# TropComplique/MultiPoseNet

Hardware: AMD Instinct MI355X
Metric: images/sec keypoint fwd+bwd+Adam @512x512 bs32/GPU (higher is better)
Workload: dtype bf16; 1 GPU; MobileNet-v1+FPN+keypoint_subnet fwd+bwd+Adam, 512x512, per-GPU batch 32; global_batch=32, parallelism=dp1, hip_graph=True, rccl_ranks=1

## Files before the change

### include/mpn.h

```cpp
#ifndef MPN_H_
#define MPN_H_

#include <stddef.h>
#include <stdint.h>

#ifdef __cplusplus
extern "C" {
#endif

#define MPN_VERSION 600

enum { MPN_F32 = 0, MPN_BF16 = 1, MPN_F16 = 2  };

enum {
    MPN_OK = 0,
    MPN_ERR_BAD_SHAPE = -1,
    MPN_ERR_BAD_DTYPE = -2,
    MPN_ERR_BAD_ALIGN = -3,
    MPN_ERR_HIP = -4,
    MPN_ERR_BAD_ARG = -5,
    MPN_ERR_WORKSPACE = -6,
    MPN_ERR_BAD_DATA = -7
};

// ... 138 lines not shown
                               mpn_stream_t stream);
int mpn_dwconv_bwd_fused_s2_apply(const void* x, const void* g, const void* y_raw, const float* w, void* dx, float* wpart, int N, int H,
                                  int W, int C, int dtype, const float* in_scale, const float* in_shift, int in_act,
                                  const float* mean, const float* invstd, float* bn_part, const void* addend, const float* ap_scale,
                                  const float* ap_shift, const float* ap_mean, const float* ap_invstd, const float* ap_k1,
                                  const float* ap_k2, int ap_act, mpn_stream_t stream);

int mpn_stem_conv_fwd(const void* images, int images_u8, const float* w, void* y, int N, int H,
                      int W, int C0, int dtype, mpn_stream_t stream);
int mpn_stem_conv_fwd_num_parts(int N, int H, int W, int C0, int dtype);
int mpn_stem_conv_fwd_stats(const void* images, int images_u8, const float* w, void* y, int N, int H, int W, int C0,
                            int dtype, float* stats_part, mpn_stream_t stream);
int mpn_stem_conv_wgrad_num_parts(int N, int H, int W);
int mpn_stem_conv_bwd_weight(const void* images, int images_u8, const void* dy, float* part, int N,
                             int H, int W, int C0, int dtype, mpn_stream_t stream);

int mpn_bilinear_up_fwd(const void* x, void* y, int N, int h, int w, int C, int upsample,
                        int y_channel_offset, int y_channels_total, int dtype,
                        const float* in_scale, const float* in_shift, int in_act,
                        mpn_stream_t stream);
int mpn_bilinear_up_bwd(const void* dy, void* dx, int N, int h, int w, int C, int upsample,
                        int y_channel_offset, int y_channels_total, int dtype, mpn_stream_t stream);
int mpn_sumpool2x2(const void* src, void* dst, int N, int h, int w, int C, int accumulate,
                   int dtype, mpn_stream_t stream);
int mpn_add_inplace(void* dst, const void* src, long long n, int dtype, mpn_stream_t stream);

int mpn_heatmap_head_fwd(const void* x, const float* w, const float* bias, long long M, int Cin,
                         int dtype, const float* in_scale, const float* in_shift, int in_act,
                         int mode, float* out, float* out_seg, mpn_stream_t stream);
int mpn_heatmap_head_bwd_num_parts(long long M);
// ... 426 lines not shown
```

### multiposenet_amd/_lib.py

```python
import ctypes
import os

_HERE = os.path.dirname(os.path.abspath(__file__))
LIB_PATH = os.environ.get("MPN_LIB") or os.path.join(_HERE, "libmpn_hip.so")

MPN_VERSION = 600
MPN_F32, MPN_BF16, MPN_F16 = 0, 1, 2
ACT_NONE, ACT_RELU, ACT_RELU6 = 0, 1, 2

_c = ctypes
_P = _c.c_void_p
_I = _c.c_int
_F = _c.c_float
_D = _c.c_double
_Z = _c.c_size_t
_L = _c.c_longlong

SIGNATURES = {
    "mpn_version": (_I, []),
    "mpn_last_error": (_I, [_c.c_char_p, _Z]),
    "mpn_heatmap_decode_workspace_bytes": (_Z, [_I]),
    "mpn_heatmap_decode": (_I, [_P, _I, _I, _I, _I, _I, _P, _F, _P, _P, _P, _P, _Z, _P]),
    "mpn_heatmap_render_workspace_bytes": (_Z, [_I]),
    "mpn_heatmap_render": (_I, [_P, _P, _P, _I, _I, _I, _I, _I, _P, _P, _Z, _P]),
# ... 38 lines not shown
    "mpn_dwconv_bwd_data_add_supported": (_I, [_I, _I, _I, _I, _I, _I]),
    "mpn_dwconv_bwd_data_add": (_I, [_P, _P, _P, _I, _I, _I, _I, _I, _I, _P, _P, _P, _P, _P, _P, _I, _P, _P]),
    "mpn_dwconv_wgrad_num_parts": (_I, [_I, _I, _I, _I, _I, _I]),
    "mpn_dwconv_bwd_weight": (_I, [_P, _P, _P, _I, _I, _I, _I, _I, _I, _P, _P, _I, _P]),
    "mpn_dwconv_bwd_fused_supported": (_I, [_I, _I, _I, _I, _I, _I]),
    "mpn_dwconv_bwd_fused": (_I, [_P, _P, _P, _P, _P, _I, _I, _I, _I, _I, _P, _P, _I, _P, _P, _P, _P]),
    "mpn_dwconv_bwd_fused_s2": (_I, [_P, _P, _P, _P, _P, _I, _I, _I, _I, _I, _P, _P, _I, _P, _P, _P, _P, _P]),
    "mpn_dwconv_bwd_fused_apply_supported": (_I, [_I, _I, _I, _I, _I, _I]),
    "mpn_dwconv_bwd_fused_apply": (_I, [_P, _P, _P, _P, _P, _P, _I, _I, _I, _I, _I, _P, _P, _I, _P, _P, _P, _P, _P, _P, _P, _P, _P, _I, _P]),
    "mpn_dwconv_bwd_fused_s2_apply": (_I, [_P, _P, _P, _P, _P, _P, _I, _I, _I, _I, _I, _P, _P, _I, _P, _P, _P, _P, _P, _P, _P, _P, _P, _P, _I, _P]),
    "mpn_stem_conv_fwd": (_I, [_P, _I, _P, _P, _I, _I, _I, _I, _I, _P]),
    "mpn_stem_conv_fwd_num_parts": (_I, [_I, _I, _I, _I, _I]),
    "mpn_stem_conv_fwd_stats": (_I, [_P, _I, _P, _P, _I, _I, _I, _I, _I, _P, _P]),
    "mpn_stem_conv_wgrad_num_parts": (_I, [_I, _I, _I]),
    "mpn_stem_conv_bwd_weight": (_I, [_P, _I, _P, _P, _I, _I, _I, _I, _I, _P]),
    "mpn_bilinear_up_fwd": (_I, [_P, _P, _I, _I, _I, _I, _I, _I, _I, _I, _P, _P, _I, _P]),
    "mpn_bilinear_up_bwd": (_I, [_P, _P, _I, _I, _I, _I, _I, _I, _I, _I, _P]),
    "mpn_sumpool2x2": (_I, [_P, _P, _I, _I, _I, _I, _I, _I, _P]),
    "mpn_add_inplace": (_I, [_P, _P, _L, _I, _P]),
    "mpn_heatmap_head_fwd": (_I, [_P, _P, _P, _L, _I, _I, _P, _P, _I, _I, _P, _P, _P]),
    "mpn_heatmap_head_bwd_num_parts": (_I, [_L]),
    "mpn_heatmap_head_bwd": (_I, [_P, _P, _P, _L, _I, _I, _P, _P, _I, _P, _P, _P]),
    "mpn_heatmap_head_bwd_bn_supported": (_I, [_I, _I]),
    "mpn_heatmap_head_bwd_bn": (_I, [_P, _P, _P, _L, _I, _I, _P, _P, _I, _P, _P, _P, _P]),
    "mpn_keypoint_loss_num_parts": (_I, [_I, _I, _I]),
    "mpn_keypoint_loss": (_I, [_P] * 9 + [_I, _I] + [_P] * 7 + [_I, _I, _I, _P]),
    "mpn_adam_prepare": (_I, [_P, _P, _D, _D, _D, _D, _D, _P]),
    "mpn_adam_step": (_I, [_P, _P, _P, _P, _L, _P, _F, _F, _F, _F, _F, _P]),
    "mpn_adam_step_cast": (_I, [_P, _P, _P, _P, _L, _P, _F, _F, _F, _F, _F, _I, _P, _P, _P, _I, _P]),
    "mpn_reduce_partials": (_I, [_P, _I, _L, _P, _I, _F, _P]),
# ... 237 lines not shown
```

### multiposenet_amd/csrc/conv_mfma.hip

```cpp
#include "common.h"
#include "pointwise.h"
#include "conv3x3.h"
#include <type_traits>
#include <string.h>

namespace {

typedef __bf16 bf16x8_t __attribute__((ext_vector_type(8)));
typedef __bf16 bf16x4_t __attribute__((ext_vector_type(4)));
typedef float f32x4_t __attribute__((ext_vector_type(4)));
typedef float f32x16_t __attribute__((ext_vector_type(16)));

template <typename T> struct Mma;
template <> struct Mma<bf16_t> {
    using Frag = bf16x8_t;
    static __device__ __forceinline__ void run(const Frag& a, const Frag& b, f32x4_t& c) {
        c = __builtin_amdgcn_mfma_f32_16x16x32_bf16(a, b, c, 0, 0, 0);
    }
};
template <> struct Mma<half_t> {
    using Frag = H16<half_t>::x8;
    static __device__ __forceinline__ void run(const Frag& a, const Frag& b, f32x4_t& c) { c = H16<half_t>::mfma(a, b, c); }
};
template <> struct Mma<float> {
// ... 600 lines not shown
    constexpr int EPS = 16 / ES;
    const int q = e / EPS, within = e - q * EPS;
    const long long dst = i - e + (long long)((q ^ b_swz(n & 15)) * EPS + within);
    out[dst] = from_f32<T>(v);
}

template <typename T>
__global__ void pack_weights_kernel(const float* __restrict__ w, T* __restrict__ out, int Cin_o, int Cout_o,
                                    int taps, int transpose, int BN, int n_tiles, int nchunk, int row_bytes,
                                    long long total_elems) {
    for (long long i = (long long)blockIdx.x * blockDim.x + threadIdx.x; i < total_elems;
         i += (long long)gridDim.x * blockDim.x)
        pack_one<T>(w, out, Cin_o, Cout_o, taps, transpose, BN, nchunk, row_bytes, i);
}

template <typename T>
__global__ void pack_weights_batched_kernel(const PackDesc* __restrict__ descs, int ndesc) {
    __shared__ int job;
    if (threadIdx.x < 64) {
        int cnt = 0;
        for (int base = 0; base < ndesc; base += 64) {
            const int i = base + (int)threadIdx.x;
            const bool le = i < ndesc && descs[i].block_begin <= (int)blockIdx.x;
            cnt += __popcll(__ballot(le));
        }
        if (threadIdx.x == 0) job = cnt - 1;
    }
    __syncthreads();
    const PackDesc d = descs[job];
    const int lb = blockIdx.x - d.block_begin;
    for (long long i = (long long)lb * blockDim.x + threadIdx.x; i < d.total_elems; i += (long long)d.block_count * blockDim.x)
        pack_one<T>(d.w, reinterpret_cast<T*>(d.out), d.Cin_o, d.Cout_o, d.taps, d.transpose, d.BN, d.nchunk, d.row_bytes, i);
}

struct PackGeom {
    int BN, n_tiles, nchunk, row_bytes;
    long long tile_bytes, total_bytes;
};

PackGeom pack_geom(int Kin, int Nout, int taps, int es, int dtype) {
    PackGeom g;
    if (dtype == MPN_BF16 && pw_gemm_eligible(Kin, Nout, taps, es)) {
        g.BN = 256; g.n_tiles = Nout / 256; g.nchunk = 1; g.row_bytes = 0;
        g.tile_bytes = 256ll * Kin * es; g.total_bytes = (long long)Nout * Kin * es;
        return g;
// ... 47 lines not shown

extern "C" size_t mpn_conv_pack_desc_bytes(void) { return sizeof(PackDesc); }

extern "C" int mpn_conv_pack_desc_fill(void* desc_host, const float* w_hwio, int Cin, int Cout, int ksize, int transpose,
                                       int dtype, void* out, int block_begin) {
    if (!(ksize == 1 || ksize == 3) || !desc_host || !w_hwio || !out) return -1;
    const int es = dtype == MPN_F32 ? 4 : 2;
    const int taps = ksize * ksize;
    const PackGeom g = pack_geom(transpose ? Cout : Cin, transpose ? Cin : Cout, taps, es, dtype);
    PackDesc d;
    d.w = w_hwio; d.out = out; d.Cin_o = Cin; d.Cout_o = Cout; d.taps = taps; d.transpose = transpose;
    d.BN = g.BN; d.n_tiles = g.n_tiles; d.nchunk = g.nchunk; d.row_bytes = g.row_bytes;
    d.total_elems = g.total_bytes / es;
    long long blocks = (d.total_elems + 4 * 256 - 1) / (4 * 256);
    if (blocks > 256) blocks = 256;
    if (blocks < 1) blocks = 1;
    d.block_begin = block_begin;
    d.block_count = (int)blocks;
    memcpy(desc_host, &d, sizeof(d));
    return (int)blocks;
}

extern "C" int mpn_conv_pack_weights_batched(const void* descs_device, int ndesc, int total_blocks, int dtype,
                                             mpn_stream_t stream) {
    MPN_REQUIRE(descs_device && ndesc > 0 && total_blocks > 0, MPN_ERR_BAD_ARG, "pack batched: bad arguments");
    MPN_REQUIRE(dtype == MPN_F32 || dtype == MPN_BF16 || dtype == MPN_F16, MPN_ERR_BAD_DTYPE, "pack batched: dtype");
    hipStream_t st = (hipStream_t)stream;
    MPN_DISPATCH_DTYPE3(dtype, (pack_weights_batched_kernel<T><<<total_blocks, 256, 0, st>>>((const PackDesc*)descs_device, ndesc)));
    MPN_LAUNCH_CHECK();
    return MPN_OK;
// ... 271 lines not shown
```

### multiposenet_amd/csrc/stem.hip

```cpp
#include "common.h"

namespace {

constexpr int kThreads = 256;
constexpr int kTile = 16;
constexpr int kIn = 2 * kTile + 1;
constexpr int kMaxC0 = 64;
constexpr int kFwdTW = 2 * kTile;

template <typename T, bool U8>
__device__ __forceinline__ void stage_patch(const void* images, float* patch, int img, int oy0, int ox0, int H, int W,
                                            int pad_t, int pad_l) {
    const int iy0 = oy0 * 2 - pad_t, ix0 = ox0 * 2 - pad_l;
    constexpr int NEL = kIn * kIn * 3;
    constexpr int PER = (NEL + kThreads - 1) / kThreads;
    float v[PER];
#pragma unroll
    for (int k = 0; k < PER; ++k) {
        const int i = threadIdx.x + k * kThreads;
        const int ch = i % 3;
        const int px = (i / 3) % kIn;
        const int py = i / (3 * kIn);
        const int iy = iy0 + py, ix = ix0 + px;
        float raw = 0.5f;
// ... 222 lines not shown
        const int r = wv * 4 + (gi >> 1), col = (gi & 1) * 16 + n;
        unsigned char* dst = otile + (r * kFwdTW + col) * orow + (4 * kg) * 2;
#pragma unroll
        for (int mb = 0; mb < MB; ++mb) {
            const acc_t c = acc[gi][mb];
            uint2 q;
            q.x = pack_bf16x2(c[0], c[1]);
            q.y = pack_bf16x2(c[2], c[3]);
            *reinterpret_cast<uint2*>(dst + mb * 32) = q;
        }
    }
    __syncthreads();
    stem_copy_out<bf16_t>(otile, orow, y, img, ty, tx, OH, OW, C0, stats_part);
}

template <typename T, bool U8>
__global__ __launch_bounds__(kThreads) void stem_wgrad_kernel(const void* __restrict__ images, const T* __restrict__ dy,
                                                              float* __restrict__ part, int N, int H, int W, int C0, int OH,
                                                              int OW, int pad_t, int pad_l, int tiles_x, int tiles_y) {
    extern __shared__ __attribute__((aligned(16))) float dyn_smem[];
    float* patch = dyn_smem;
    float* g = dyn_smem + kIn * kIn * 3 + 1;
    const int ncq = C0 / 8;
    const int tpp = 9 * ncq;
    const int nphase = min(kThreads / tpp, kTile * kTile / 27);
    const int ph = threadIdx.x / tpp;
    const int r = threadIdx.x - ph * tpp;
    const int pos = r / ncq, cq = r - pos * ncq;
    const int ky = pos / 3, kx = pos - ky * 3;
    const bool active = ph < nphase;
    f32x2_t acc[3][4];
#pragma unroll
    for (int a = 0; a < 3; ++a)
#pragma unroll
        for (int j = 0; j < 4; ++j) acc[a][j] = (f32x2_t){0.f, 0.f};
    const int nout = 27 * C0;
    const int ntiles = N * tiles_y * tiles_x;
    constexpr int NEL = kIn * kIn * 3;
    constexpr int PER = (NEL + kThreads - 1) / kThreads;
    constexpr int VE = Vec16<T>::N;
    constexpr int DPER = kTile * kTile * (kMaxC0 / VE) / kThreads;
    const int vpp = C0 / VE;
    const int ndv = kTile * kTile * vpp / kThreads;
    float pv[PER];
    Vec16<T> dvv[DPER];
    unsigned pmask = 0u, dmask = 0u;

    auto load_tile = [&](int t) {
        const int tx = t % tiles_x;
        const int t2 = t / tiles_x;
        const int ty = t2 % tiles_y;
        const int img = t2 / tiles_y;
        const int oy0 = ty * kTile, ox0 = tx * kTile;
        const int iy0 = oy0 * 2 - pad_t, ix0 = ox0 * 2 - pad_l;
        pmask = 0u;
        dmask = 0u;
#pragma unroll
        for (int k = 0; k < PER; ++k) {
            const int i = threadIdx.x + k * kThreads;
            const int ch = i % 3;
            const int px = (i / 3) % kIn;
            const int py = i / (3 * kIn);
            const int iy = iy0 + py, ix = ix0 + px;
            const bool ok = i < NEL && iy >= 0 && iy < H && ix >= 0 && ix < W;
            const long long off = ok ? (((long long)img * H + iy) * W + ix) * 3 + ch : 0;
            pv[k] = U8 ? (float)reinterpret_cast<const unsigned char*>(images)[off] * (1.0f / 255.0f)
                       : reinterpret_cast<const float*>(images)[off];
            pmask |= (ok ? 1u : 0u) << k;
        }
#pragma unroll
        for (int k = 0; k < DPER; ++k) {
            if (k < ndv) {
                const int i = threadIdx.x + k * kThreads;
                const int vq = i % vpp, px = i / vpp;
                const int oy = oy0 + px / kTile, ox = ox0 + px % kTile;
                const bool ok = oy < OH && ox < OW;
                dvv[k].load(dy + (ok ? (((long long)img * OH + oy) * OW + ox) * C0 + vq * VE : 0));
                dmask |= (ok ? 1u : 0u) << k;
            }
        }
    };
    auto commit_tile = [&]() {
#pragma unroll
        for (int k = 0; k < PER; ++k) {
            const int i = threadIdx.x + k * kThreads;
            if (i < NEL) patch[i] = ((pmask >> k) & 1u) ? 2.0f * pv[k] - 1.0f : 0.0f;
        }
#pragma unroll
        for (int k = 0; k < DPER; ++k) {
            if (k < ndv) {
                const int i = threadIdx.x + k * kThreads;
                const int vq = i % vpp, px = i / vpp;
                float f[VE];
                dvv[k].unpack(f);
                const bool ok = (dmask >> k) & 1u;
#pragma unroll
                for (int j = 0; j < VE; j += 4)
                    *reinterpret_cast<float4*>(g + px * C0 + vq * VE + j) =
                        ok ? make_float4(f[j], f[j + 1], f[j + 2], f[j + 3]) : make_float4(0.f, 0.f, 0.f, 0.f);
            }
        }
    };

    int t = blockIdx.x;
    if (t < ntiles) {
        load_tile(t);
        commit_tile();
    }
// ... 27 lines not shown
        for (int a = 0; a < 3; ++a)
#pragma unroll
            for (int j = 0; j < 4; ++j) {
                g[ph * nout + (pos * 3 + a) * C0 + cq * 8 + 2 * j] = acc[a][j].x;
                g[ph * nout + (pos * 3 + a) * C0 + cq * 8 + 2 * j + 1] = acc[a][j].y;
            }
    }
    __syncthreads();
    for (int o = threadIdx.x; o < nout; o += kThreads) {
        float s = 0.f;
        for (int q = 0; q < nphase; ++q) s += g[q * nout + o];
        part[(long long)blockIdx.x * nout + o] = s;
    }
}

template <bool U8, int MB>
__global__ __launch_bounds__(kThreads) void stem_wgrad_mfma_kernel(const void* __restrict__ images, const bf16_t* __restrict__ dy,
                                                                   float* __restrict__ part, int N, int H, int W, int OH, int OW,
                                                                   int pad_t, int pad_l, int tiles_x, int tiles_y) {
    typedef H16<bf16_t> HT;
    typedef HT::x8 x8;
    typedef HT::x4 x4;
    typedef HT::acc_t acc_t;
    constexpr int C0 = 16 * MB;
    constexpr int DRS = C0 * 2 + 16;
    extern __shared__ __attribute__((aligned(16))) unsigned char stem_smem[];
    float* patch = reinterpret_cast<float*>(stem_smem);
    unsigned char* dimg = stem_smem + kPR * kPS * sizeof(float);
    const int ntiles = N * tiles_y * tiles_x;
    const int lane = threadIdx.x & 63, wv = threadIdx.x >> 6;
    const int n = lane & 15, kg = lane >> 4, q = n >> 2, pq = n & 3;
    constexpr int VPP = C0 / 8;
    constexpr int DV = kTile * kFwdTW * VPP / kThreads;
    float pv[kPR];
    uint4 dv[DV];
    unsigned long long pmask = 0ull;
    unsigned dmask = 0u;
    const int p_pc = threadIdx.x < kPC ? threadIdx.x : 0;
    auto load_tile = [&](int t) __attribute__((always_inline)) {
        const int tx = t % tiles_x;
        const int t2 = t / tiles_x;
        const int ty = t2 % tiles_y;
        const int img = t2 / tiles_y;
        const int iy0 = ty * kTile * 2 - pad_t, ix0 = tx * kFwdTW * 2 - pad_l;
        pmask = 0ull;
        dmask = 0u;
        int tid = threadIdx.x;
        asm volatile("" : "+v"(tid));
        {
            const int ix = ix0 + p_pc / 3;
            const bool col_ok = tid < kPC && ix >= 0 && ix < W;
            const long long base = ((long long)img * H * W + ix0) * 3 + p_pc;
#pragma unroll
            for (int py = 0; py < kPR; ++py) {
                const int iy = iy0 + py;
                const bool ok = col_ok && iy >= 0 && iy < H;
                const long long off = ok ? base + (long long)iy * W * 3 : 0;
                pv[py] = U8 ? (float)reinterpret_cast<const unsigned char*>(images)[off] * (1.0f / 255.0f)
                            : reinterpret_cast<const float*>(images)[off];
                pmask |= (unsigned long long)(ok ? 1u : 0u) << py;
            }
        }
#pragma unroll
        for (int k = 0; k < DV; ++k) {
            const int i = tid + k * kThreads;
            const int vq = i % VPP, px = i / VPP;
            const int oy = ty * kTile + px / kFwdTW, ox = tx * kFwdTW + px % kFwdTW;
            const bool ok = oy < OH && ox < OW;
            dv[k] = *reinterpret_cast<const uint4*>(dy + (ok ? (((long long)img * OH + oy) * OW + ox) * C0 + vq * 8 : 0));
            dmask |= (ok ? 1u : 0u) << k;
        }
    };
    auto commit_tile = [&]() __attribute__((always_inline)) {
        int tid = threadIdx.x;
        asm volatile("" : "+v"(tid));
        if (tid < kPC) {
#pragma unroll
            for (int py = 0; py < kPR; ++py)
                patch[py * kPS + p_pc] = ((pmask >> py) & 1ull) ? 2.0f * pv[py] - 1.0f : 0.0f;
        }
#pragma unroll
        for (int k = 0; k < DV; ++k) {
            const int i = tid + k * kThreads;
            const int vq = i % VPP, px = i / VPP;
            *reinterpret_cast<uint4*>(dimg + px * DRS + vq * 16) = ((dmask >> k) & 1u) ? dv[k] : make_uint4(0u, 0u, 0u, 0u);
        }
    };
    int kbase[2];
    bool kval[2];
#pragma unroll
    for (int nb = 0; nb < 2; ++nb) {
        const int k = nb * 16 + n;
        kval[nb] = k < 27;
        kbase[nb] = kval[nb] ? (k / 9) * kPS + (k % 9) : 0;
    }
    acc_t acc[MB][2];
#pragma unroll
    for (int mb = 0; mb < MB; ++mb)
#pragma unroll
        for (int nb = 0; nb < 2; ++nb) acc[mb][nb] = (acc_t){0.f, 0.f, 0.f, 0.f};
// ... 48 lines not shown
        for (int nb = 0; nb < 2; ++nb)
            *reinterpret_cast<float4*>(red + ((wv * (MB * 2) + mb * 2 + nb) * 64 + lane) * 4) =
                make_float4(acc[mb][nb][0], acc[mb][nb][1], acc[mb][nb][2], acc[mb][nb][3]);
    __syncthreads();
    for (int o = threadIdx.x; o < 27 * C0; o += kThreads) {
        const int k = o / C0, co = o - k * C0;
        const int nb = k >> 4, nn = k & 15, mb = co >> 4, m = co & 15;
        const int ln = (m >> 2) * 16 + nn, e = m & 3;
        float sacc = 0.f;
#pragma unroll
        for (int w4 = 0; w4 < 4; ++w4) sacc += red[((w4 * (MB * 2) + mb * 2 + nb) * 64 + ln) * 4 + e];
        part[(long long)blockIdx.x * (27 * C0) + o] = sacc;
    }
}

template <bool U8, int MB>
int launch_stem_wgrad_mfma(int grid, hipStream_t st, const void* images, const void* dy, float* part, int N, int H, int W, int OH,
                           int OW, int pt, int pl, int tiles_x, int tiles_y) {
    constexpr int sm = kPR * kPS * (int)sizeof(float) + kTile * kFwdTW * (16 * MB * 2 + 16);
    static mpn_attr_mask_t attr_mask{0};
    MPN_HIP(mpn_ensure_dynamic_lds((const void*)stem_wgrad_mfma_kernel<U8, MB>, sm, &attr_mask));
    stem_wgrad_mfma_kernel<U8, MB><<<grid, kThreads, sm, st>>>(images, (const bf16_t*)dy, part, N, H, W, OH, OW, pt, pl, tiles_x, tiles_y);
    return MPN_OK;
}

void same_pad(int size, int* out, int* pad_before) {
    *out = (size + 1) / 2;
    int total = (*out - 1) * 2 + 3 - size;
    if (total < 0) total = 0;
    *pad_before = total / 2;
}

int check(int N, int H, int W, int C0, int dtype) {
    MPN_REQUIRE(dtype == MPN_F32 || dtype == MPN_BF16, MPN_ERR_BAD_DTYPE, "stem: dtype %d", dtype);
    const int ve = dtype == MPN_F32 ? 4 : 8;
    MPN_REQUIRE(N > 0 && H > 0 && W > 0, MPN_ERR_BAD_SHAPE, "stem: bad shape");
    MPN_REQUIRE(C0 > 0 && C0 <= kMaxC0 && C0 % ve == 0, MPN_ERR_BAD_SHAPE, "stem: C0 (%d) must be <= %d and a multiple of %d",
                C0, kMaxC0, ve);
// ... 58 lines not shown
        } else {
            if (sm > 48 * 1024)
                MPN_HIP(hipFuncSetAttribute((const void*)stem_fwd_kernel<T, false>, hipFuncAttributeMaxDynamicSharedMemorySize, sm));
            stem_fwd_kernel<T, false><<<grid, kThreads, sm, st>>>(images, w, (T*)y, N, H, W, C0, OH, OW, pt, pl, tiles_x, tiles_y, stats_part);
        }
    });
    MPN_LAUNCH_CHECK();
    return MPN_OK;
}

extern "C" int mpn_stem_conv_wgrad_num_parts(int N, int H, int W) {
    const int ntiles = N * (((H + 1) / 2 + kTile - 1) / kTile) * (((W + 1) / 2 + kTile - 1) / kTile);
    return ntiles < 512 ? ntiles : 512;
}

extern "C" int mpn_stem_conv_bwd_weight(const void* images, int images_u8, const void* dy, float* part, int N, int H, int W,
                                        int C0, int dtype, mpn_stream_t stream) {
    if (int rc = check(N, H, W, C0, dtype)) return rc;
    MPN_REQUIRE(images && dy && part, MPN_ERR_BAD_ARG, "stem_wgrad: null pointer");
    int OH, OW, pt, pl;
    same_pad(H, &OH, &pt);
    same_pad(W, &OW, &pl);
    const int tiles_y = (OH + kTile - 1) / kTile, tiles_x = (OW + kTile - 1) / kTile;
    const int grid = mpn_stem_conv_wgrad_num_parts(N, H, W);
    hipStream_t st = (hipStream_t)stream;
    MPN_REQUIRE(C0 % 8 == 0, MPN_ERR_BAD_SHAPE, "stem_wgrad: C0 must be a multiple of 8");
    if (dtype == MPN_BF16 && C0 % 16 == 0) {
        const int tx32 = (OW + kFwdTW - 1) / kFwdTW;
        int rc;
#define MPN_STEM_WG(MB)                                                                                                         \
    rc = images_u8 ? launch_stem_wgrad_mfma<true, MB>(grid, st, images, dy, part, N, H, W, OH, OW, pt, pl, tx32, tiles_y)       \
                   : launch_stem_wgrad_mfma<false, MB>(grid, st, images, dy, part, N, H, W, OH, OW, pt, pl, tx32, tiles_y)
        switch (C0 / 16) {
            case 1: MPN_STEM_WG(1); break;
            case 2: MPN_STEM_WG(2); break;
            case 3: MPN_STEM_WG(3); break;
            default: MPN_STEM_WG(4); break;
        }
#undef MPN_STEM_WG
        if (rc) return rc;
        MPN_LAUNCH_CHECK();
        return MPN_OK;
    }
    const size_t sm = (size_t)(kIn * kIn * 3 + 1 + kTile * kTile * C0) * sizeof(float);
    MPN_REQUIRE(sm <= 64 * 1024, MPN_ERR_BAD_SHAPE, "stem_wgrad: C0 too large");
    MPN_DISPATCH_DTYPE(dtype, {
        if (images_u8)
            stem_wgrad_kernel<T, true><<<grid, kThreads, sm, st>>>(images, (const T*)dy, part, N, H, W, C0, OH, OW, pt, pl, tiles_x, tiles_y);
        else
            stem_wgrad_kernel<T, false><<<grid, kThreads, sm, st>>>(images, (const T*)dy, part, N, H, W, C0, OH, OW, pt, pl, tiles_x, tiles_y);
    });
    MPN_LAUNCH_CHECK();
    return MPN_OK;
}
```

### multiposenet_amd/net.py

```python
import math
import os
from collections import OrderedDict

import numpy as np
import torch

from . import _lib, ops
from ._lib import ACT_NONE, ACT_RELU, ACT_RELU6
from .model_state import ModelState, _Arena, is_trainable, resolve_device

NUM_KEYPOINTS = 17
DOWNSAMPLE = 4
DIVISOR = 128
DEPTH = 128
STRIDES_AND_FILTERS = [(1, 64), (2, 128), (1, 128), (2, 256), (1, 256), (2, 512), (1, 512), (1, 512),
                       (1, 512), (1, 512), (1, 512), (2, 1024), (1, 1024)]
FEATURE_BLOCKS = {3: "c2", 5: "c3", 11: "c4", 13: "c5"}


def depth(x, depth_multiplier):
    return max(int(x * depth_multiplier), 8)


def variable_shapes(depth_multiplier=1.0):
# ... 132 lines not shown
                               conv2=self._conv(s + "/conv2/kernel"), bn2=self._bn(s + "/bn2", ACT_RELU))
        self.final_conv = self._conv("final_conv3x3/kernel")
        self.final_bn = self._bn("final_bn", ACT_RELU)
        self.concat_scale = torch.ones(4 * DEPTH, dtype=torch.float32, device=self.device)
        self.concat_shift = torch.zeros(4 * DEPTH, dtype=torch.float32, device=self.device)
        self.phi[2]["bn2"].scale = self.concat_scale[:DEPTH]
        self.phi[2]["bn2"].shift = self.concat_shift[:DEPTH]
        self.concat_affine = ops.Affine(self.concat_scale, self.concat_shift, ACT_RELU)
        self.heat_w, self.heat_b = self.vars["heatmaps/kernel"], self.vars["heatmaps/bias"]
        ok, nk, _ = self._train_arena.offsets["heatmaps/kernel"]
        ob, nb, _ = self._train_arena.offsets["heatmaps/bias"]
        assert ob == ok + nk, "heatmaps/kernel and heatmaps/bias must be adjacent in the arena"
        self._head_grad = self.grad[ok:ob + nb]
        self.fuse_dw_bn = True
        self.fuse_dw_apply = True
        self.fuse_conv_bn = True
        self._l2 = None
        self._wd = None
        self.cache_inference_affine = False
        self._infer_clean = False
        self.fuse_stem_stats = True
        self._build_pack_table()
        self.all_bn = [self.stem_bn] + [b[k] for b in self.blocks for k in ("dw_bn", "pw_bn")] + \
            [self.p_bn[l] for l in (2, 3, 4, 5)] + [self.phi[l][k] for l in (2, 3, 4, 5) for k in ("bn1", "bn2")] + [self.final_bn]

    def _build_pack_table(self):
        import ctypes
        lib = ops._lib.lib()
        nb = lib.mpn_conv_pack_desc_bytes()
        jobs = [(c, t) for c in self.convs for t in (0, 1)]
# ... 368 lines not shown
        if phase == 1:
            dA, reduced, lateral_added = g["c"]["c5"], g.get("c5_reduced", 0), False
            rng = range(last, first - 1, -1)
        else:
            dA, reduced, lateral_added = g["bb_chain"]
            rng = range(first - 1, -1, -1)
        for i in rng:
            feature = FEATURE_BLOCKS.get(self.blocks[i]["i"])
            if feature in ("c2", "c3", "c4") and not lateral_added:
                ops.add_inplace(dA, g["c"][feature])
            dY, applied = self._backward_pointwise(b, g, sp, slab, i, dA, reduced, raw=i == last, fold=self._dw_folds_apply(b, g, i))
            dA, reduced, lateral_added = self._backward_depthwise(b, g, sp, slab, i, dY, apply=not applied)
        if phase == 1:
            g["bb_chain"] = (dA, reduced, lateral_added)
            return
        ops.bn_backward(self.stem_bn, g["stem"], b["stem"], sp, reduced_parts=reduced)
        ops.stem_conv_bwd_weight(images, g["stem"], self.stem_dw, slab[id(self.stem_dw)], reduce=False)

    def _dw_lateral(self, g, i):
        return g["c"][FEATURE_BLOCKS[self.blocks[i - 1]["i"]]] if i > 0 and self.blocks[i - 1]["i"] in FEATURE_BLOCKS else None

    def _dw_walks_fused(self, b, g, i):
        s, (N, _, _, C) = self.blocks[i]["stride"], b["dw"][i].shape
        return (self.fuse_dw_bn and (s == 2 or self._dw_lateral(g, i) is None)
                and ops.dwconv_bwd_fused_supported(N, *b["hw"][i], C, s, self.dtype))

    def _dw_folds_apply(self, b, g, i):
        s, (N, _, _, C) = self.blocks[i]["stride"], b["dw"][i].shape
        return (self.fuse_dw_apply and self._dw_walks_fused(b, g, i)
                and ops.dwconv_bwd_fused_apply_supported(N, *b["hw"][i], C, s, self.dtype))

    def _backward_pointwise(self, b, g, sp, slab, i, dA, reduced, raw, fold=False):
# ... 59 lines not shown
```

### multiposenet_amd/ops.py

```python
import ctypes
from collections import namedtuple

import torch

from . import _lib
from ._lib import ACT_NONE, ACT_RELU, ACT_RELU6, call, ptr, stream_ptr

BN_MOMENTUM = 0.95
BN_EPSILON = 1e-3

LAUNCH_JOBS_ALONE = False

Affine = namedtuple("Affine", ["scale", "shift", "act"])


def _f32(n, dev):
    return torch.empty(n, dtype=torch.float32, device=dev)


def _check_nhwc(x, name="x"):
    if x.dim() != 4 or not x.is_contiguous():
        raise ValueError(f"{name} must be a contiguous NHWC tensor, got shape {tuple(x.shape)}")
    if x.dtype not in (torch.float32, torch.bfloat16):
        raise ValueError(f"{name}: unsupported dtype {x.dtype}")
# ... 531 lines not shown
        raise ValueError("images must be float32 in [0,1] or uint8")
    N, H, W, _ = images.shape
    if out is None:
        out = torch.empty((N, (H + 1) // 2, (W + 1) // 2, c0), dtype=dtype, device=images.device)
    if stats_part is not None:
        rows = stem_conv_fwd_num_parts(N, H, W, c0, dtype)
        if rows <= 0 or stats_part.numel() < rows * 2 * c0:
            raise ValueError("stem_conv_fwd: fused statistics not available for this shape, or slab too small")
        call("mpn_stem_conv_fwd_stats", ptr(images), int(u8), ptr(w), ptr(out), N, H, W, c0, _lib.dtype_code(dtype),
             ptr(stats_part), stream_ptr())
        return out
    call("mpn_stem_conv_fwd", ptr(images), int(u8), ptr(w), ptr(out), N, H, W, c0, _lib.dtype_code(dtype), stream_ptr())
    return out


def stem_conv_bwd_weight(images, dy, dw_out, part=None, reduce=True):
    N, H, W, _ = images.shape
    c0 = dy.shape[3]
    nparts = _lib.lib().mpn_stem_conv_wgrad_num_parts(N, H, W)
    if part is None:
        part = _f32(nparts * 27 * c0, dy.device)
    call("mpn_stem_conv_bwd_weight", ptr(images), int(images.dtype == torch.uint8), ptr(dy), ptr(part), N, H, W, c0,
         _lib.dtype_code(dy.dtype), stream_ptr())
    if reduce:
        call("mpn_reduce_partials", ptr(part), nparts, 27 * c0, ptr(dw_out), 0, 1.0, stream_ptr())
    return dw_out


def bilinear_up_fwd(x, upsample, out, channel_offset, affine=None):
    N, h, w, C = x.shape
    sc, sh, act = _aff(affine)
    call("mpn_bilinear_up_fwd", ptr(x), ptr(out), N, h, w, C, upsample, channel_offset, out.shape[3],
         _lib.dtype_code(x.dtype), sc, sh, act, stream_ptr())
    return out


def bilinear_up_bwd(dy, upsample, channel_offset, C, out=None):
    N, OH, OW, ctot = dy.shape
# ... 193 lines not shown
```

Baseline: 4295 images/s.

## Fold stem BN-backward apply into stem weight-grad load; tile weight packing via LDS

The stem batch-norm backward no longer runs a separate apply pass over the stem gradient. The stem weight-gradient kernels now read the raw pre-BN output alongside dy and apply the ReLU mask and BN correction on load, which saves one read/write pass over a large full-resolution activation. Separately, bf16 weight packing now stages 32-row groups through shared memory so that global loads and stores are vectorised and coalesced. The cost is extra register pressure and an additional y load inside the stem wgrad kernel.

Measured after the change: 4320 images/s (median of 6 runs). No clear change (+0.6%).

```diff
diff --git a/include/mpn.h b/include/mpn.h
--- a/include/mpn.h
+++ b/include/mpn.h
@@ -176,6 +176,10 @@
 int mpn_stem_conv_wgrad_num_parts(int N, int H, int W);
 int mpn_stem_conv_bwd_weight(const void* images, int images_u8, const void* dy, float* part, int N,
                              int H, int W, int C0, int dtype, mpn_stream_t stream);
+int mpn_stem_conv_bwd_weight_apply_supported(int N, int H, int W, int C0, int dtype);
+int mpn_stem_conv_bwd_weight_apply(const void* images, int images_u8, const void* g, const void* y_raw, float* part, int N, int H,
+                                   int W, int C0, int dtype, const float* ap_scale, const float* ap_shift, const float* ap_mean,
+                                   const float* ap_invstd, const float* ap_k1, const float* ap_k2, int ap_act, mpn_stream_t stream);
 
 int mpn_bilinear_up_fwd(const void* x, void* y, int N, int h, int w, int C, int upsample,
                         int y_channel_offset, int y_channels_total, int dtype,
diff --git a/multiposenet_amd/_lib.py b/multiposenet_amd/_lib.py
--- a/multiposenet_amd/_lib.py
+++ b/multiposenet_amd/_lib.py
@@ -76,6 +76,8 @@
     "mpn_stem_conv_fwd_stats": (_I, [_P, _I, _P, _P, _I, _I, _I, _I, _I, _P, _P]),
     "mpn_stem_conv_wgrad_num_parts": (_I, [_I, _I, _I]),
     "mpn_stem_conv_bwd_weight": (_I, [_P, _I, _P, _P, _I, _I, _I, _I, _I, _P]),
+    "mpn_stem_conv_bwd_weight_apply_supported": (_I, [_I, _I, _I, _I, _I]),
+    "mpn_stem_conv_bwd_weight_apply": (_I, [_P, _I, _P, _P, _P, _I, _I, _I, _I, _I, _P, _P, _P, _P, _P, _P, _I, _P]),
     "mpn_bilinear_up_fwd": (_I, [_P, _P, _I, _I, _I, _I, _I, _I, _I, _I, _P, _P, _I, _P]),
     "mpn_bilinear_up_bwd": (_I, [_P, _P, _I, _I, _I, _I, _I, _I, _I, _I, _P]),
     "mpn_sumpool2x2": (_I, [_P, _P, _I, _I, _I, _I, _I, _I, _P]),
diff --git a/multiposenet_amd/csrc/conv_mfma.hip b/multiposenet_amd/csrc/conv_mfma.hip
--- a/multiposenet_amd/csrc/conv_mfma.hip
+++ b/multiposenet_amd/csrc/conv_mfma.hip
@@ -638,8 +638,107 @@
         pack_one<T>(w, out, Cin_o, Cout_o, taps, transpose, BN, nchunk, row_bytes, i);
 }
 
+constexpr int kPackGroupK = 32;
+__host__ __device__ inline int pack_group_rows(int BN, int row_bytes) { return row_bytes == 0 ? 64 : BN; }
+
+template <typename T>
+__device__ __forceinline__ void pack_group(const PackDesc& d, int grp, float* __restrict__ tile) {
+    static_assert(sizeof(T) == 2, "tiled packing: 16-bit images");
+    const int Kin = d.transpose ? d.Cout_o : d.Cin_o, Nout = d.transpose ? d.Cin_o : d.Cout_o;
+    const int NB = pack_group_rows(d.BN, d.row_bytes);
+    const int pitch = NB + 4;
+    int tap, cbase, nbase, g = grp;
+    long long dst0 = (long long)grp * NB * kPackGroupK;
+    int dst_pitch = kPackGroupK;
+    if (d.row_bytes == -2) {
+        const int ks = g % 2; g /= 2;
+        const int ky = g % 3; g /= 3;
+        const int kx = g % 3; g /= 3;
+        const int chunk = g % d.nchunk; g /= d.nchunk;
+        tap = ky * 3 + kx; cbase = chunk * 64 + ks * 32; nbase = g * 64;
+    } else if (d.row_bytes < 0) {
+        const int ky = g % 3; g /= 3;
+        const int ks = g % 2; g /= 2;
+        const int kx = g % 3; g /= 3;
+        const int chunk = g % d.nchunk; g /= d.nchunk;
+        tap = ky * 3 + kx; cbase = chunk * 64 + ks * 32; nbase = g * 128;
+    } else if (d.row_bytes == 0) {
+        const int kblocks = Kin / kPackGroupK;
+        const int kb = g % kblocks; g /= kblocks;
+        tap = 0; cbase = kb * kPackGroupK; nbase = g * 64;
+        dst0 = (long long)nbase * Kin + cbase;
+        dst_pitch = Kin;
+    } else {
+        const int stages_per_tap = d.row_bytes >> 7;
+        const int ks = g % 2; g /= 2;
+        const int st = g % stages_per_tap; g /= stages_per_tap;
+        tap = g % d.taps; g /= d.taps;
+        const int chunk = g % d.nchunk; g /= d.nchunk;
+        cbase = chunk * (d.row_bytes / 2) + (st * 2 + ks) * kPackGroupK; nbase = g * d.BN;
+    }
+    const bool swizzled = d.row_bytes != 0;
+    const bool c3 = d.row_bytes < 0;
+    const float* __restrict__ w = d.w;
+    const bool vec_ok = (d.Cout_o & 3) == 0 && (reinterpret_cast<uintptr_t>(w) & 15u) == 0;
+    T* __restrict__ out = reinterpret_cast<T*>(d.out);
+    const int tid = threadIdx.x, nthreads = blockDim.x;
+    if (!d.transpose) {
+        const long long src0 = (long long)tap * d.Cin_o * d.Cout_o;
+        const int f4_per_row = NB / 4;
+        for (int f = tid; f < kPackGroupK * f4_per_row; f += nthreads) {
+            const int row = f / f4_per_row, c4 = f - row * f4_per_row;
+            const int c = cbase + row, co = nbase + c4 * 4;
+            float4 v = make_float4(0.f, 0.f, 0.f, 0.f);
+            if (c < Kin) {
+                const float* src = w + src0 + (long long)c * d.Cout_o + co;
+                if (vec_ok && co + 3 < Nout) v = *reinterpret_cast<const float4*>(src);
+                else {
+                    if (co < Nout) v.x = src[0];
+                    if (co + 1 < Nout) v.y = src[1];
+                    if (co + 2 < Nout) v.z = src[2];
+                    if (co + 3 < Nout) v.w = src[3];
+                }
+            }
+            *reinterpret_cast<float4*>(tile + row * pitch + c4 * 4) = v;
+        }
+        __syncthreads();
+    }
+    for (int vi = tid; vi < NB * 4; vi += nthreads) {
+        const int n = vi >> 2, qd = vi & 3;
+        const int q = swizzled ? (qd ^ (c3 ? mpn_c3::swz(n & 15) : b_swz(n & 15))) : qd;
+        float f[8];
+        if (!d.transpose) {
+#pragma unroll
+            for (int j = 0; j < 8; ++j) f[j] = tile[(q * 8 + j) * pitch + n];
+        } else {
+            const int co = nbase + n, c0 = cbase + q * 8;
+#pragma unroll
+            for (int j = 0; j < 8; ++j) f[j] = 0.f;
+            if (co < Nout) {
+                const float* src = w + ((long long)(d.taps - 1 - tap) * d.Cin_o + co) * d.Cout_o + c0;
+                if (vec_ok && c0 + 7 < Kin) {
+                    const float4 a = *reinterpret_cast<const float4*>(src), b = *reinterpret_cast<const float4*>(src + 4);
+                    f[0] = a.x; f[1] = a.y; f[2] = a.z; f[3] = a.w; f[4] = b.x; f[5] = b.y; f[6] = b.z; f[7] = b.w;
+                } else {
+#pragma unroll
+                    for (int j = 0; j < 8; ++j)
+                        if (c0 + j < Kin) f[j] = src[j];
+                }
+            }
+        }
+        T t[8];
+#pragma unroll
+        for (int j = 0; j < 8; ++j) t[j] = from_f32<T>(f[j]);
+        uint4 o;
+        __builtin_memcpy(&o, t, 16);
+        *reinterpret_cast<uint4*>(out + dst0 + (long long)n * dst_pitch + qd * 8) = o;
+    }
+    if (!d.transpose) __syncthreads();
+}
+
 template <typename T>
 __global__ void pack_weights_batched_kernel(const PackDesc* __restrict__ descs, int ndesc) {
+    __shared__ __attribute__((aligned(16))) float tile[sizeof(T) == 2 ? kPackGroupK * (128 + 4) : 4];
     __shared__ int job;
     if (threadIdx.x < 64) {
         int cnt = 0;
@@ -653,6 +752,13 @@
     __syncthreads();
     const PackDesc d = descs[job];
     const int lb = blockIdx.x - d.block_begin;
+    if constexpr (sizeof(T) == 2) {
+        if ((reinterpret_cast<uintptr_t>(d.out) & 15u) == 0) {
+            const int ngroups = (int)(d.total_elems / (pack_group_rows(d.BN, d.row_bytes) * kPackGroupK));
+            for (int grp = lb; grp < ngroups; grp += d.block_count) pack_group<T>(d, grp, tile);
+            return;
+        }
+    }
     for (long long i = (long long)lb * blockDim.x + threadIdx.x; i < d.total_elems; i += (long long)d.block_count * blockDim.x)
         pack_one<T>(d.w, reinterpret_cast<T*>(d.out), d.Cin_o, d.Cout_o, d.taps, d.transpose, d.BN, d.nchunk, d.row_bytes, i);
 }
@@ -730,6 +836,10 @@
     d.total_elems = g.total_bytes / es;
     long long blocks = (d.total_elems + 4 * 256 - 1) / (4 * 256);
     if (blocks > 256) blocks = 256;
+    if (es == 2) {
+        blocks = d.total_elems / (pack_group_rows(g.BN, g.row_bytes) * kPackGroupK);
+        if (blocks > 512) blocks = 512;
+    }
     if (blocks < 1) blocks = 1;
     d.block_begin = block_begin;
     d.block_count = (int)blocks;
diff --git a/multiposenet_amd/csrc/stem.hip b/multiposenet_amd/csrc/stem.hip
--- a/multiposenet_amd/csrc/stem.hip
+++ b/multiposenet_amd/csrc/stem.hip
@@ -1,8 +1,7 @@
-#include "common.h"
+#include "dwconv_walk.h"
 
 namespace {
 
-constexpr int kThreads = 256;
 constexpr int kTile = 16;
 constexpr int kIn = 2 * kTile + 1;
 constexpr int kMaxC0 = 64;
@@ -260,10 +259,55 @@
     stem_copy_out<bf16_t>(otile, orow, y, img, ty, tx, OH, OW, C0, stats_part);
 }
 
-template <typename T, bool U8>
+struct StemApplyArgs {
+    const void* y;
+    const float* scale; const float* shift; const float* mean; const float* invstd; const float* k1; const float* k2;
+    int act;
+};
+struct StemDyApply {
+    DyApply<bf16_t> a[2];
+    f32x2_t sh[4];
+    float lo, hi;
+    __device__ __forceinline__ void load(const StemApplyArgs& p, int c0) {
+#pragma unroll
+        for (int h = 0; h < 2; ++h) {
+            a[h].load(p.scale, p.mean, p.invstd, p.k1, p.k2, c0 + 4 * h);
+            const float4 h4 = *reinterpret_cast<const float4*>(p.shift + c0 + 4 * h);
+            sh[2 * h] = (f32x2_t){h4.x, h4.y};
+            sh[2 * h + 1] = (f32x2_t){h4.z, h4.w};
+        }
+        lo = (p.act != MPN_ACT_NONE) ? 0.f : -INFINITY;
+        hi = (p.act == MPN_ACT_RELU6) ? 6.f : INFINITY;
+    }
+    __device__ __forceinline__ uint4 apply(const uint4& g, const uint4& y, unsigned elem) const {
+        const unsigned gw[4] = {g.x, g.y, g.z, g.w}, yw[4] = {y.x, y.y, y.z, y.w};
+        unsigned ow[4];
+#pragma unroll
+        for (int h = 0; h < 2; ++h) {
+            const Raw4<bf16_t> gr = {make_uint2(gw[2 * h], gw[2 * h + 1])}, yr = {make_uint2(yw[2 * h], yw[2 * h + 1])};
+            float f[4];
+            raw_unpack(gr, f);
+            f32x2_t y01, y23;
+            raw_unpack2(yr, y01, y23);
+            const f32x2_t p01 = __builtin_elementwise_fma(y01, a[h].sc01, sh[2 * h]);
+            const f32x2_t p23 = __builtin_elementwise_fma(y23, a[h].sc23, sh[2 * h + 1]);
+            f[0] = (p01.x > lo && p01.x < hi) ? f[0] : 0.f;
+            f[1] = (p01.y > lo && p01.y < hi) ? f[1] : 0.f;
+            f[2] = (p23.x > lo && p23.x < hi) ? f[2] : 0.f;
+            f[3] = (p23.y > lo && p23.y < hi) ? f[3] : 0.f;
+            a[h].apply(f, yr, elem);
+            ow[2 * h] = (__float_as_uint(f[0]) >> 16) | (__float_as_uint(f[1]) & 0xffff0000u);
+            ow[2 * h + 1] = (__float_as_uint(f[2]) >> 16) | (__float_as_uint(f[3]) & 0xffff0000u);
+        }
+        return make_uint4(ow[0], ow[1], ow[2], ow[3]);
+    }
+};
+
+template <typename T, bool U8, bool AP = false>
 __global__ __launch_bounds__(kThreads) void stem_wgrad_kernel(const void* __restrict__ images, const T* __restrict__ dy,
                                                               float* __restrict__ part, int N, int H, int W, int C0, int OH,
-                                                              int OW, int pad_t, int pad_l, int tiles_x, int tiles_y) {
+                                                              int OW, int pad_t, int pad_l, int tiles_x, int tiles_y,
+                                                              const StemApplyArgs ap) {
     extern __shared__ __attribute__((aligned(16))) float dyn_smem[];
     float* patch = dyn_smem;
     float* g = dyn_smem + kIn * kIn * 3 + 1;
@@ -290,7 +334,8 @@
     const int ndv = kTile * kTile * vpp / kThreads;
     float pv[PER];
     Vec16<T> dvv[DPER];
-    unsigned pmask = 0u, dmask = 0u;
+    Vec16<T> yvv[AP ? DPER : 1];
+    unsigned pmask = 0u, dmask = 0u, umask = 0u;
 
     auto load_tile = [&](int t) {
         const int tx = t % tiles_x;
@@ -321,8 +366,13 @@
                 const int vq = i % vpp, px = i / vpp;
                 const int oy = oy0 + px / kTile, ox = ox0 + px % kTile;
                 const bool ok = oy < OH && ox < OW;
-                dvv[k].load(dy + (ok ? (((long long)img * OH + oy) * OW + ox) * C0 + vq * VE : 0));
+                const long long off = ok ? (((long long)img * OH + oy) * OW + ox) * C0 + vq * VE : 0;
+                dvv[k].load(dy + off);
                 dmask |= (ok ? 1u : 0u) << k;
+                if constexpr (AP) {
+                    yvv[k].load(reinterpret_cast<const T*>(ap.y) + off);
+                    umask = (umask & ~(3u << (2 * k))) | (((unsigned)(off >> 11) & 3u) << (2 * k));
+                }
             }
         }
     };
@@ -338,6 +388,11 @@
                 const int i = threadIdx.x + k * kThreads;
                 const int vq = i % vpp, px = i / vpp;
                 float f[VE];
+                if constexpr (AP) {
+                    StemDyApply sa;
+                    sa.load(ap, 0);
+                    dvv[k].raw = sa.apply(dvv[k].raw, yvv[k].raw, ((umask >> (2 * k)) & 3u) << 11);
+                }
                 dvv[k].unpack(f);
                 const bool ok = (dmask >> k) & 1u;
 #pragma unroll
@@ -395,10 +450,11 @@
     }
 }
 
-template <bool U8, int MB>
+template <bool U8, int MB, bool AP = false>
 __global__ __launch_bounds__(kThreads) void stem_wgrad_mfma_kernel(const void* __restrict__ images, const bf16_t* __restrict__ dy,
                                                                    float* __restrict__ part, int N, int H, int W, int OH, int OW,
-                                                                   int pad_t, int pad_l, int tiles_x, int tiles_y) {
+                                                                   int pad_t, int pad_l, int tiles_x, int tiles_y,
+                                                                   const StemApplyArgs ap) {
     typedef H16<bf16_t> HT;
     typedef HT::x8 x8;
     typedef HT::x4 x4;
@@ -415,8 +471,12 @@
     constexpr int DV = kTile * kFwdTW * VPP / kThreads;
     float pv[kPR];
     uint4 dv[DV];
+    uint4 yv[AP ? DV : 1];
+    static_assert(!AP || kThreads % VPP == 0, "apply on load: a thread keeps its channel vector");
+    StemDyApply sa;
+    if constexpr (AP) sa.load(ap, ((int)threadIdx.x % VPP) * 8);
     unsigned long long pmask = 0ull;
-    unsigned dmask = 0u;
+    unsigned dmask = 0u, umask = 0u;
     const int p_pc = threadIdx.x < kPC ? threadIdx.x : 0;
     auto load_tile = [&](int t) __attribute__((always_inline)) {
         const int tx = t % tiles_x;
@@ -426,6 +486,7 @@
         const int iy0 = ty * kTile * 2 - pad_t, ix0 = tx * kFwdTW * 2 - pad_l;
         pmask = 0ull;
         dmask = 0u;
+        umask = 0u;
         int tid = threadIdx.x;
         asm volatile("" : "+v"(tid));
         {
@@ -448,8 +509,13 @@
             const int vq = i % VPP, px = i / VPP;
             const int oy = ty * kTile + px / kFwdTW, ox = tx * kFwdTW + px % kFwdTW;
             const bool ok = oy < OH && ox < OW;
-            dv[k] = *reinterpret_cast<const uint4*>(dy + (ok ? (((long long)img * OH + oy) * OW + ox) * C0 + vq * 8 : 0));
+            const long long off = ok ? (((long long)img * OH + oy) * OW + ox) * C0 + vq * 8 : 0;
+            dv[k] = *reinterpret_cast<const uint4*>(dy + off);
             dmask |= (ok ? 1u : 0u) << k;
+            if constexpr (AP) {
+                yv[k] = *reinterpret_cast<const uint4*>(reinterpret_cast<const bf16_t*>(ap.y) + off);
+                umask |= ((unsigned)(off >> 11) & 3u) << (2 * k);
+            }
         }
     };
     auto commit_tile = [&]() __attribute__((always_inline)) {
@@ -464,7 +530,9 @@
         for (int k = 0; k < DV; ++k) {
             const int i = tid + k * kThreads;
             const int vq = i % VPP, px = i / VPP;
-            *reinterpret_cast<uint4*>(dimg + px * DRS + vq * 16) = ((dmask >> k) & 1u) ? dv[k] : make_uint4(0u, 0u, 0u, 0u);
+            uint4 v = dv[k];
+            if constexpr (AP) v = sa.apply(dv[k], yv[k], ((umask >> (2 * k)) & 3u) << 11);
+            *reinterpret_cast<uint4*>(dimg + px * DRS + vq * 16) = ((dmask >> k) & 1u) ? v : make_uint4(0u, 0u, 0u, 0u);
         }
     };
     int kbase[2];
@@ -543,14 +611,17 @@
     }
 }
 
-template <bool U8, int MB>
+template <bool U8, int MB, bool AP>
 int launch_stem_wgrad_mfma(int grid, hipStream_t st, const void* images, const void* dy, float* part, int N, int H, int W, int OH,
-                           int OW, int pt, int pl, int tiles_x, int tiles_y) {
+                           int OW, int pt, int pl, int tiles_x, int tiles_y, const StemApplyArgs& ap) {
+    if constexpr (AP && kThreads % (2 * MB) != 0) return MPN_ERR_BAD_SHAPE;
+    else {
     constexpr int sm = kPR * kPS * (int)sizeof(float) + kTile * kFwdTW * (16 * MB * 2 + 16);
     static mpn_attr_mask_t attr_mask{0};
-    MPN_HIP(mpn_ensure_dynamic_lds((const void*)stem_wgrad_mfma_kernel<U8, MB>, sm, &attr_mask));
-    stem_wgrad_mfma_kernel<U8, MB><<<grid, kThreads, sm, st>>>(images, (const bf16_t*)dy, part, N, H, W, OH, OW, pt, pl, tiles_x, tiles_y);
+    MPN_HIP(mpn_ensure_dynamic_lds((const void*)stem_wgrad_mfma_kernel<U8, MB, AP>, sm, &attr_mask));
+    stem_wgrad_mfma_kernel<U8, MB, AP><<<grid, kThreads, sm, st>>>(images, (const bf16_t*)dy, part, N, H, W, OH, OW, pt, pl, tiles_x, tiles_y, ap);
     return MPN_OK;
+    }
 }
 
 void same_pad(int size, int* out, int* pad_before) {
@@ -639,23 +710,59 @@
     return ntiles < 512 ? ntiles : 512;
 }
 
+namespace {
+int stem_bwd_weight(const void* images, int images_u8, const void* dy, float* part, int N, int H, int W, int C0, int dtype,
+                    const StemApplyArgs* ap, mpn_stream_t stream);
+}
+
 extern "C" int mpn_stem_conv_bwd_weight(const void* images, int images_u8, const void* dy, float* part, int N, int H, int W,
                                         int C0, int dtype, mpn_stream_t stream) {
     if (int rc = check(N, H, W, C0, dtype)) return rc;
     MPN_REQUIRE(images && dy && part, MPN_ERR_BAD_ARG, "stem_wgrad: null pointer");
+    return stem_bwd_weight(images, images_u8, dy, part, N, H, W, C0, dtype, nullptr, stream);
+}
+
+extern "C" int mpn_stem_conv_bwd_weight_apply_supported(int N, int H, int W, int C0, int dtype) {
+    return dtype == MPN_BF16 && N > 0 && H > 0 && W > 0 && C0 >= 8 && C0 <= kMaxC0 && C0 % 8 == 0 && kThreads % (C0 / 8) == 0;
+}
+
+extern "C" int mpn_stem_conv_bwd_weight_apply(const void* images, int images_u8, const void* g, const void* y_raw, float* part, int N,
+                                              int H, int W, int C0, int dtype, const float* ap_scale, const float* ap_shift,
+                                              const float* ap_mean, const float* ap_invstd, const float* ap_k1, const float* ap_k2,
+                                              int ap_act, mpn_stream_t stream) {
+    MPN_REQUIRE(images && g && y_raw && part && ap_scale && ap_shift && ap_mean && ap_invstd && ap_k1 && ap_k2, MPN_ERR_BAD_ARG,
+                "stem_wgrad_apply: null pointer");
+    MPN_REQUIRE(mpn_stem_conv_bwd_weight_apply_supported(N, H, W, C0, dtype), MPN_ERR_BAD_SHAPE,
+                "stem_wgrad_apply: not supported for N = %d, H = %d, W = %d, C0 = %d, dtype %d (mpn_stem_conv_bwd_weight_apply_supported)",
+                N, H, W, C0, dtype);
+    MPN_REQUIRE(ap_act == MPN_ACT_NONE || ap_act == MPN_ACT_RELU || ap_act == MPN_ACT_RELU6, MPN_ERR_BAD_ARG,
+                "stem_wgrad_apply: activation %d", ap_act);
+    MPN_REQUIRE(mpn_aligned16(g) && mpn_aligned16(y_raw) && mpn_aligned16(ap_scale) && mpn_aligned16(ap_shift) && mpn_aligned16(ap_mean) &&
+                    mpn_aligned16(ap_invstd) && mpn_aligned16(ap_k1) && mpn_aligned16(ap_k2),
+                MPN_ERR_BAD_ALIGN, "stem_wgrad_apply: g, y_raw and the batch-norm vectors must be 16-byte aligned");
+    const StemApplyArgs ap = {y_raw, ap_scale, ap_shift, ap_mean, ap_invstd, ap_k1, ap_k2, ap_act};
+    return stem_bwd_weight(images, images_u8, g, part, N, H, W, C0, dtype, &ap, stream);
+}
+
+namespace {
+int stem_bwd_weight(const void* images, int images_u8, const void* dy, float* part, int N, int H, int W, int C0, int dtype,
+                    const StemApplyArgs* ap, mpn_stream_t stream) {
     int OH, OW, pt, pl;
     same_pad(H, &OH, &pt);
     same_pad(W, &OW, &pl);
     const int tiles_y = (OH + kTile - 1) / kTile, tiles_x = (OW + kTile - 1) / kTile;
     const int grid = mpn_stem_conv_wgrad_num_parts(N, H, W);
     hipStream_t st = (hipStream_t)stream;
+    const StemApplyArgs none = {nullptr, nullptr, nullptr, nullptr, nullptr, nullptr, nullptr, MPN_ACT_NONE};
     MPN_REQUIRE(C0 % 8 == 0, MPN_ERR_BAD_SHAPE, "stem_wgrad: C0 must be a multiple of 8");
     if (dtype == MPN_BF16 && C0 % 16 == 0) {
         const int tx32 = (OW + kFwdTW - 1) / kFwdTW;
         int rc;
 #define MPN_STEM_WG(MB)                                                                                                         \
-    rc = images_u8 ? launch_stem_wgrad_mfma<true, MB>(grid, st, images, dy, part, N, H, W, OH, OW, pt, pl, tx32, tiles_y)       \
-                   : launch_stem_wgrad_mfma<false, MB>(grid, st, images, dy, part, N, H, W, OH, OW, pt, pl, tx32, tiles_y)
+    rc = ap ? (images_u8 ? launch_stem_wgrad_mfma<true, MB, true>(grid, st, images, dy, part, N, H, W, OH, OW, pt, pl, tx32, tiles_y, *ap)       \
+                         : launch_stem_wgrad_mfma<false, MB, true>(grid, st, images, dy, part, N, H, W, OH, OW, pt, pl, tx32, tiles_y, *ap))     \
+            : (images_u8 ? launch_stem_wgrad_mfma<true, MB, false>(grid, st, images, dy, part, N, H, W, OH, OW, pt, pl, tx32, tiles_y, none)     \
+                         : launch_stem_wgrad_mfma<false, MB, false>(grid, st, images, dy, part, N, H, W, OH, OW, pt, pl, tx32, tiles_y, none))
         switch (C0 / 16) {
             case 1: MPN_STEM_WG(1); break;
             case 2: MPN_STEM_WG(2); break;
@@ -669,12 +776,21 @@
     }
     const size_t sm = (size_t)(kIn * kIn * 3 + 1 + kTile * kTile * C0) * sizeof(float);
     MPN_REQUIRE(sm <= 64 * 1024, MPN_ERR_BAD_SHAPE, "stem_wgrad: C0 too large");
+    if (ap) {
+        if (images_u8)
+            stem_wgrad_kernel<bf16_t, true, true><<<grid, kThreads, sm, st>>>(images, (const bf16_t*)dy, part, N, H, W, C0, OH, OW, pt, pl, tiles_x, tiles_y, *ap);
+        else
+            stem_wgrad_kernel<bf16_t, false, true><<<grid, kThreads, sm, st>>>(images, (const bf16_t*)dy, part, N, H, W, C0, OH, OW, pt, pl, tiles_x, tiles_y, *ap);
+        MPN_LAUNCH_CHECK();
+        return MPN_OK;
+    }
     MPN_DISPATCH_DTYPE(dtype, {
         if (images_u8)
-            stem_wgrad_kernel<T, true><<<grid, kThreads, sm, st>>>(images, (const T*)dy, part, N, H, W, C0, OH, OW, pt, pl, tiles_x, tiles_y);
+            stem_wgrad_kernel<T, true><<<grid, kThreads, sm, st>>>(images, (const T*)dy, part, N, H, W, C0, OH, OW, pt, pl, tiles_x, tiles_y, none);
         else
-            stem_wgrad_kernel<T, false><<<grid, kThreads, sm, st>>>(images, (const T*)dy, part, N, H, W, C0, OH, OW, pt, pl, tiles_x, tiles_y);
+            stem_wgrad_kernel<T, false><<<grid, kThreads, sm, st>>>(images, (const T*)dy, part, N, H, W, C0, OH, OW, pt, pl, tiles_x, tiles_y, none);
     });
     MPN_LAUNCH_CHECK();
     return MPN_OK;
 }
+}
diff --git a/multiposenet_amd/net.py b/multiposenet_amd/net.py
--- a/multiposenet_amd/net.py
+++ b/multiposenet_amd/net.py
@@ -170,6 +170,7 @@
         self._head_grad = self.grad[ok:ob + nb]
         self.fuse_dw_bn = True
         self.fuse_dw_apply = True
+        self.fuse_stem_apply = True
         self.fuse_conv_bn = True
         self._l2 = None
         self._wd = None
@@ -568,8 +569,11 @@
         if phase == 1:
             g["bb_chain"] = (dA, reduced, lateral_added)
             return
-        ops.bn_backward(self.stem_bn, g["stem"], b["stem"], sp, reduced_parts=reduced)
-        ops.stem_conv_bwd_weight(images, g["stem"], self.stem_dw, slab[id(self.stem_dw)], reduce=False)
+        N, H, W, _ = images.shape
+        fold = self.fuse_stem_apply and ops.stem_conv_bwd_weight_apply_supported(N, H, W, g["stem"].shape[3], self.dtype)
+        ops.bn_backward(self.stem_bn, g["stem"], b["stem"], sp, reduced_parts=reduced, apply=not fold)
+        ops.stem_conv_bwd_weight(images, g["stem"], self.stem_dw, slab[id(self.stem_dw)], reduce=False,
+                                 apply_bn=self.stem_bn if fold else None, y_raw=b["stem"] if fold else None)
 
     def _dw_lateral(self, g, i):
         return g["c"][FEATURE_BLOCKS[self.blocks[i - 1]["i"]]] if i > 0 and self.blocks[i - 1]["i"] in FEATURE_BLOCKS else None
diff --git a/multiposenet_amd/ops.py b/multiposenet_amd/ops.py
--- a/multiposenet_amd/ops.py
+++ b/multiposenet_amd/ops.py
@@ -569,14 +569,26 @@
     return out
 
 
-def stem_conv_bwd_weight(images, dy, dw_out, part=None, reduce=True):
+def stem_conv_bwd_weight_apply_supported(N, H, W, c0, dtype):
+    return _lib.lib().mpn_stem_conv_bwd_weight_apply_supported(N, H, W, c0, _lib.dtype_code(dtype)) == 1
+
+
+def stem_conv_bwd_weight(images, dy, dw_out, part=None, reduce=True, apply_bn=None, y_raw=None):
     N, H, W, _ = images.shape
     c0 = dy.shape[3]
     nparts = _lib.lib().mpn_stem_conv_wgrad_num_parts(N, H, W)
     if part is None:
         part = _f32(nparts * 27 * c0, dy.device)
-    call("mpn_stem_conv_bwd_weight", ptr(images), int(images.dtype == torch.uint8), ptr(dy), ptr(part), N, H, W, c0,
-         _lib.dtype_code(dy.dtype), stream_ptr())
+    if apply_bn is not None:
+        bn = apply_bn
+        if y_raw is None or y_raw.shape != dy.shape or y_raw.dtype != dy.dtype or not y_raw.is_contiguous() or not dy.is_contiguous():
+            raise ValueError("stem_conv_bwd_weight: y_raw must be a contiguous tensor of dy's shape and type")
+        call("mpn_stem_conv_bwd_weight_apply", ptr(images), int(images.dtype == torch.uint8), ptr(dy), ptr(y_raw), ptr(part), N, H, W,
+             c0, _lib.dtype_code(dy.dtype), ptr(bn.scale), ptr(bn.shift), ptr(bn.mean), ptr(bn.invstd), ptr(bn.k1), ptr(bn.k2),
+             int(bn.act), stream_ptr())
+    else:
+        call("mpn_stem_conv_bwd_weight", ptr(images), int(images.dtype == torch.uint8), ptr(dy), ptr(part), N, H, W, c0,
+             _lib.dtype_code(dy.dtype), stream_ptr())
     if reduce:
         call("mpn_reduce_partials", ptr(part), nparts, 27 * c0, ptr(dw_out), 0, 1.0, stream_ptr())
     return dw_out
```
